# leejeongho3214/LightHand

Measured on AMD Instinct MI355X. Metric: images/sec/GPU (256×256, bs=64) train+infer; EPE/AUC parity, higher is better.
Workload: dtype bf16; 1 GPU; SimpleBaseline-ResNet50 256x256 training step (fwd + JointsMSELoss + argmax decode + bwd + Adam), batch 64/GPU, 21 joints, random init (seed 9001), hipGraph replay; global_batch=64, parallelism=dp1

## Files before the change

include/lighthand_hip.h:

```cpp
#ifndef LIGHTHAND_HIP_H
#define LIGHTHAND_HIP_H

#include <stddef.h>
#include <stdint.h>

#ifdef __cplusplus
extern "C" {
#endif

typedef enum { LH_F32 = 0, LH_BF16 = 1, LH_F16 = 2 } lh_dtype;

typedef enum {
    LH_OK = 0,
    LH_ERR_ARG = -1,
    LH_ERR_HIP = -2,
    LH_ERR_UNSUPPORTED = -3
} lh_status;

int lh_version(void);
const char* lh_last_error(void);
int lh_dtype_size(int dtype);

int lh_image_to_nhwc4(const float* nchw, void* out, int n, int h, int w, int pad, int wp,
                      int dtype, void* stream);
int lh_image_u8_to_nhwc4(const unsigned char* hwc, void* out, int n, int hs, int ws, int h, int w, int pad, int wp,
                         const float* mean3, const float* std3, int dtype, void* stream);
size_t lh_image_jitter_workspace_bytes(int n);
int lh_image_u8_jitter_to_nhwc4(const unsigned char* hwc, void* out, int n, int hs, int ws, int h, int w, int pad, int wp,
                                const float* mean3, const float* std3, const float* factors_dev, const int* order_dev,
                                void* workspace, int dtype, void* stream);
int lh_image_u8_warp_to_nhwc4(const unsigned char* hwc, void* out, int n, int hs, int ws, int h, int w, int pad, int wp,
                              const float* mean3, const float* std3, const float* inv_dev,
                              const float* factors_dev, const int* order_dev, void* workspace, int dtype, void* stream);
int lh_affine_points(const float* pts, int pstride, const float* fwd_dev, float* out, int ostride, int b, int j, void* stream);
int lh_nhwc4_mirror(void* img, int n, int h, int w, int pad, int wp, int dtype, void* stream);
int lh_nhwc_to_nchw_f32(const void* nhwc, float* nchw, int n, int h, int w, int c, int c_stride,
                        int dtype, void* stream);
int lh_nchw_f32_to_nhwc(const float* nchw, void* nhwc, int n, int h, int w, int c, int c_stride,
                        int dtype, void* stream);

int lh_pack_weight(const float* w, void* out, size_t* bytes, int n_out, int n_in,
                   long so, long si, long sr, long ss, int ntaps, const int* taps_rs,
                   int dtype, void* stream);

typedef struct {
    const float* w;
    void* out;
    int n_out, n_in, ntaps, pad_;
    long so, si, sr, ss;
    signed char r[64];
    signed char s[64];
} lh_pack_item;
int lh_pack_chunk_elems(void);
int lh_pack_weights_multi(const lh_pack_item* items_dev, const int* chunk_item_dev, const long* chunk_start_dev,
                          int n_chunks, int dtype, void* stream);

typedef struct {
    void* out;
    int row_is_d1, ntaps, kpad, pad_;
    int taps[16];
} lh_pack_out;
typedef struct {
    const float* w;
    int d0, d1, rs, npacks;
    lh_pack_out packs[5];
} lh_pack_conv;
int lh_pack_weights_tiled(const lh_pack_conv* convs_dev, const int* chunk_conv_dev, const int* chunk_t0_dev,
                          const int* chunk_t1_dev, int n_chunks, int max_rs, int dtype, void* stream);

typedef struct {
    int n, hi, wi;
    int in_pix_stride;
    int k_run;
    int ho, wo;
    int sh, sw;
    int cout;
    int OH, OW;
    int osh, osw, ooh, oow;
    int out_pix_stride;
    int ntaps;
    int relu;
    signed char dh[64];
    signed char dw[64];
    int cfg[8];
} lh_igemm_desc;

int lh_igemm(const lh_igemm_desc* d, const void* in, const void* wpack, void* out,
             const void* addend, const void* addend_mask, const float* bias, const float* scale, const float* shift,
             float* stats, int dtype, void* stream);
typedef struct {
    const void* x;
    const float* mean;
    const float* invstd;
    const float* scale;
    const float* shift;
    float* partial;
    const void* mask;
    const void* x2;
    const float* mean2;
    const float* invstd2;
    float* partial2;
} lh_bn_bwd_gate;
int lh_igemm_gated_rows(const lh_igemm_desc* d, int dtype, int nterms);
int lh_igemm_gated(const lh_igemm_desc* d, const void* in, const void* wpack, void* out, const void* addend, const void* addend_mask,
                   const lh_bn_bwd_gate* gate, int dtype, void* stream);
int lh_igemm_phases_rows(const lh_igemm_desc* const* descs, int nphase, int dtype);
int lh_igemm_phases(const lh_igemm_desc* const* descs, int nphase, const void* in, const void* const* wpacks,
                    void* out, const void* addend, const void* addend_mask, const float* bias, const float* scale,
                    const float* shift, float* stats, int dtype, void* stream);
typedef struct {
    const void* w;
    size_t w_row_bytes;
    const float* bias;
    float* out;
    int n_out;
} lh_head;
int lh_igemm_phases_head(const lh_igemm_desc* const* descs, int nphase, const void* in, const void* const* wpacks,
                         const float* scale, const float* shift, const lh_head* head, int dtype, void* stream);
int lh_igemm_tile(const lh_igemm_desc* d, int dtype, int* bm, int* bp, int* ring);
int lh_igemm_config(const lh_igemm_desc* d, int dtype, int* cfg5);
int lh_igemm_candidates(const lh_igemm_desc* d, int dtype, int* cfgs, int max);
int lh_wgrad_rowfold(const lh_igemm_desc* d, int rows, const void* x, const void* dy, int dy_pix_stride,
                     int n_out, float* slab, int dtype, void* stream);
int lh_wgrad_tile(const lh_igemm_desc* d, int n_out, int n_in, int dtype, int* bo, int* bi, int* nsplit, int* ring);
int lh_wgrad_candidates(const lh_igemm_desc* d, int n_out, int n_in, int dtype, int* out, int max);
typedef struct {
    const lh_igemm_desc* d; const void* in; const void* wpack; void* out; const void* addend; const void* addend_mask;
    const float* bias; const float* scale; const float* shift; float* stats;
} lh_igemm_call;
int lh_igemm_multi(const lh_igemm_call* calls, int n, int dtype, void* stream);
int lh_igemm_stats_rows(const lh_igemm_desc* d, int dtype);

size_t lh_wgrad_slab_bytes(const lh_igemm_desc* d, int n_out, int n_in, int dtype);
int lh_wgrad(const lh_igemm_desc* d, const void* x, const void* dy, int dy_pix_stride,
             int n_out, int n_in, float* slab, int dtype, void* stream);
int lh_wgrad_reduce(const lh_igemm_desc* d, const float* slab, float* grad, int n_out, int n_in,
                    long so, long si, long sr, long ss, const int* taps_rs, int accumulate,
                    int dtype, void* stream);
size_t lh_wgrad_workspace_bytes(const lh_igemm_desc* d, int n_out, int n_in, int dtype);
typedef struct {
    const lh_igemm_desc* d; int rows; const void* x; const void* dy; int dy_pix_stride, n_out, n_in; void* workspace; float* grad;
    long so, si, sr, ss; const int* taps_rs; int accumulate;
} lh_wgrad_call;
int lh_wgrad_fused_multi(const lh_wgrad_call* calls, int n, int dtype, void* stream);
int lh_wgrad_fused(const lh_igemm_desc* d, int rows, const void* x, const void* dy, int dy_pix_stride, int n_out, int n_in,
                   void* workspace, float* grad, long so, long si, long sr, long ss, const int* taps_rs, int accumulate,
                   int dtype, void* stream);
typedef struct {
    int bo, bi, kps, depth;
    int n_problems, n_fold;
    int n_items, n_fold_items;
    int fold_lds, target_stages, nsplit_max;
    int run_parts;
    size_t off_items, off_fold_args, off_fold_items, table_bytes, workspace_bytes;
} lh_wgrad_table_info;
int lh_wgrad_table_build(const lh_wgrad_call* calls, int n, int dtype, const int* cfg4, int target_stages, void* workspace,
                         void* host_blob, size_t host_bytes, lh_wgrad_table_info* info);
int lh_wgrad_table_run(const void* table, const lh_wgrad_table_info* info, int dtype, void* stream);


int lh_bn_stats(const void* y, int m, int c, float* stats, int* rows_out, int dtype, void* stream);
int lh_bn_stats_rows(int m, int c);
size_t lh_bn_stats_slab_bytes(int rows, int c);
int lh_bn_finalize(const float* stats, int rows, int count, int c, const float* gamma,
                   const float* beta, float* running_mean, float* running_var,
                   long long* num_batches_tracked, float momentum, float eps, float* scale,
                   float* shift, float* save_mean, float* save_invstd, void* stream);
typedef struct {
    const float* stats; int rows, count, c; const float* gamma; const float* beta; float* running_mean; float* running_var;
    long long* num_batches_tracked; float momentum, eps; float* scale; float* shift; float* save_mean; float* save_invstd;
} lh_bn_finalize_call;
int lh_bn_finalize_multi(const lh_bn_finalize_call* calls, int n, void* stream);
int lh_bn_eval_affine(const float* gamma, const float* beta, const float* running_mean,
                      const float* running_var, float eps, int c, float* scale, float* shift,
                      void* stream);

typedef struct {
    const void* x[4];
    const float* scale[4];
    const float* shift[4];
    int log2up[4];
    int nterms;
    int relu;
    void* relu_mask;
    const lh_bn_finalize_call* fin[4];
    const void* l2_touch;
    size_t l2_touch_bytes;
} lh_fuse_desc;
int lh_fuse_fwd(const lh_fuse_desc* d, void* out, int n, int h, int w, int c, int dtype, void* stream);
typedef struct { const lh_fuse_desc* d; void* out; int n, h, w, c; } lh_fuse_fwd_call;
int lh_fuse_fwd_multi(const lh_fuse_fwd_call* calls, int n, int dtype, void* stream);

typedef struct {
    const void* dout;
    const void* out;
    const void* x[4];
    const float* scale[4];
    const float* shift[4];
    const float* save_mean[4];
    const float* save_invstd[4];
    void* dx[4];
    float* dgamma[4];
    float* dbeta[4];
    int log2up[4];
    int accumulate[4];
    int nterms;
    int relu;
    const void* relu_mask;
    int strips_cap;
    const float* pre_partial;
    int pre_rows;
    const void* l2_touch;
    size_t l2_touch_bytes;
    const float* pre_partial2;
} lh_fuse_bwd_desc;
size_t lh_fuse_bwd_workspace_bytes(int n, int h, int w, int c);
int lh_fuse_bwd(const lh_fuse_bwd_desc* d, int n, int h, int w, int c, void* workspace,
                int dtype, void* stream);
typedef struct { const lh_fuse_bwd_desc* d; int n, h, w, c; void* workspace; } lh_fuse_bwd_call;
int lh_fuse_bwd_multi(const lh_fuse_bwd_call* calls, int n, int dtype, void* stream);

int lh_stem_pool(const void* img, int n, int hp, int wp, const void* wpack, const float* bias, const float* scale,
                 const float* shift, void* out, int conv_h, int conv_w, int relu, int dtype, void* stream);

typedef struct { int n, h, w, cin, mid, cout; } lh_bottleneck_desc;
int lh_bottleneck_infer(const lh_bottleneck_desc* d, const void* x, const void* w1, const void* w2, const void* w3,
                        const float* s1, const float* b1, const float* s2, const float* b2, const float* s3, const float* b3,
                        const void* residual, void* out, int dtype, void* stream);

int lh_stem_conv_rows(int n, int conv_h, int conv_w);
int lh_stem_conv(const void* img, int n, int hp, int wp, const void* wpack, void* out, float* stats, int conv_h, int conv_w,
                 int dtype, void* stream);

int lh_maxpool3x3s2_fwd(const void* x, void* out, unsigned char* idx, int n, int h, int w, int c,
                        int dtype, void* stream);
int lh_maxpool3x3s2_bwd(const void* dout, const unsigned char* idx, void* dx, int n, int h, int w,
                        int c, int dtype, void* stream);
int lh_maxpool3x3s2_bwd_gated_rows(int n, int h, int w, int c, int dtype);
int lh_maxpool3x3s2_bwd_gated(const void* dout, const unsigned char* idx, void* dx, const lh_bn_bwd_gate* gate, int n, int h, int w,
                              int c, int dtype, void* stream);
int lh_bn_relu_maxpool3x3s2_fwd(const void* x, const float* scale, const float* shift, void* out, unsigned char* idx, int n,
                                int h, int w, int c, int dtype, void* stream);

int lh_gaussian_target(const float* joints, int jstride, const float* patch, int radius,
                       float* target, int b, int j, int size, void* stream);
int lh_gaussian_target_alt(const float* points, int pstride, const float* patch, int sigma,
                           float* target, int b, int j, int res, void* stream);
size_t lh_mse_workspace_bytes(long numel);
int lh_mse_heatmap(const float* pred, const float* target, long numel, float* loss, float* grad,
                   const float* grad_scale, void* workspace, void* stream);
int lh_gaussian_target_w(const float* joints, int jstride, const float* vis, int vstride, const float* patch, int radius,
                         float* target, float* weight, int b, int j, int size, void* stream);
int lh_gaussian_target_sub(const float* joints, int jstride, const float* vis, int vstride, int radius, float sigma,
                           float* target, float* weight, int b, int j, int size, void* stream);
size_t lh_joints_mse_workspace_bytes(int b, int j);
int lh_joints_mse(const float* pred, const float* target, const float* weight, int b, int j, int hw, int topk, float* loss,
                  float* joint_loss, float* grad, const float* grad_scale, void* workspace, void* stream);
int lh_heatmap_argmax(const float* heatmaps, int bj, int h, int w, float scale, float* preds,
                      float* maxvals, int* idx, void* stream);
int lh_heatmap_soft_argmax(const float* heatmaps, int bj, int h, int w, float beta, float scale, float* preds,
                           void* stream);
int lh_heatmap_refine(const float* heatmaps, const int* idx, const float* maxvals, int bj, int h, int w,
                      float scale, float* preds, void* stream);
size_t lh_integral_l1_workspace_bytes(int b, int j);
int lh_integral_l1(const float* heatmaps, const float* joints, int jstride, const float* weight, int b, int j, int h, int w,
                   float beta, float scale, float lambda, float* preds, float* joint_loss, float* loss, int add_to_loss,
                   float* grad, int add_to_grad, const float* grad_scale, void* workspace, void* stream);
int lh_heatmap_dark(const float* heatmaps, const int* idx, const float* maxvals, int bj, int h, int w, int blur_kernel,
                    float scale, float* preds, void* stream);
int lh_heatmap_flip_merge(const float* a, const float* m, int bj, int h, int w, int shift, float scale, float* merged,
                          float* preds, float* maxvals, int* idx, void* stream);

int lh_keypoint_metrics(const float* pred, const float* gt, int gt_stride, int b, int j, float T, int* wrong,
                        float* epe, void* stream);

int lh_adam_step(float* param, const float* grad, float* exp_avg, float* exp_avg_sq, long numel,
                 const double* hyper, int* step, float* derived, float grad_scale, void* stream);
int lh_adam_tick(const double* hyper, int* step, float* derived, void* stream);
int lh_adam_apply(float* param, const float* grad, float* exp_avg, float* exp_avg_sq, long numel, const float* derived,
                  float grad_scale, void* stream);

int lh_amp_check_blocks(void);
int lh_amp_check(const float* grad, long numel, int* partial, void* stream);
int lh_amp_update(const int* partial, const double* amp_hyper, float* scale, int* growth_tracker, int* found_inf, int* skipped,
                  float* inv, double extra, const double* hyper, int* step, float* derived, void* stream);
int lh_adam_apply_guarded(float* param, const float* grad, float* exp_avg, float* exp_avg_sq, long numel, const float* derived,
                          const int* found_inf, const float* inv, void* stream);

size_t lh_channel_sum_workspace_bytes(int c);
int lh_channel_sum_nchw(const float* x, int n, int c, int hw, float* out, void* workspace, void* stream);

int lh_channel_sum_nhwc(const void* x, long pixels, int c, int pix_stride, float* out, void* workspace, int dtype, void* stream);

int lh_pck_curve(const float* pred, const float* gt, int gt_stride, const float* bb, int n, int j, const double* thr,
                 int nthr, unsigned long long* counts, unsigned long long* nvis, double* diff_row, void* stream);

typedef struct lh_comm lh_comm;
int lh_comm_unique_id(void* id128);
int lh_comm_init(lh_comm** comm, int rank, int nranks, const void* id128);
int lh_comm_allreduce_sum(lh_comm* comm, void* buf, size_t count, int dtype, void* stream);
int lh_comm_reduce_scatter_sum(lh_comm* comm, const void* send, void* recv, size_t count, int dtype, void* stream);
int lh_comm_allgather(lh_comm* comm, const void* send, void* recv, size_t count, int dtype, void* stream);
int lh_comm_alltoall(lh_comm* comm, const void* send, void* recv, size_t count, int dtype, void* stream);
int lh_comm_size(const lh_comm* comm, int* rank, int* nranks);
int lh_comm_destroy(lh_comm* comm);

int lh_copy_strided_f32(float* dst, const float* src, const int* shape4, const long* dst_strides4, const long* src_strides4,
                        void* stream);


int lh_cast_f32_bf16(float* f32, void* b16, long n, int to_f32, void* stream);

int lh_sum_chunks(const void* in, void* out, int rows, long len, int dtype, void* stream);

#ifdef __cplusplus
}
#endif
#endif
```

lighthand_amd/_lib.py:

```python
import ctypes as C
import os

_HERE = os.path.dirname(os.path.abspath(__file__))
LIB_PATH = os.environ.get("LH_LIB_PATH") or os.path.join(_HERE, "liblighthand_hip.so")

LH_F32, LH_BF16, LH_F16 = 0, 1, 2


class LightHandError(RuntimeError):
    pass


class IgemmDesc(C.Structure):
    _fields_ = [("n", C.c_int), ("hi", C.c_int), ("wi", C.c_int), ("in_pix_stride", C.c_int),
                ("k_run", C.c_int), ("ho", C.c_int), ("wo", C.c_int), ("sh", C.c_int), ("sw", C.c_int),
                ("cout", C.c_int), ("OH", C.c_int), ("OW", C.c_int), ("osh", C.c_int), ("osw", C.c_int),
                ("ooh", C.c_int), ("oow", C.c_int), ("out_pix_stride", C.c_int), ("ntaps", C.c_int),
                ("relu", C.c_int), ("dh", C.c_byte * 64), ("dw", C.c_byte * 64), ("cfg", C.c_int * 8)]


class BnFinalizeCall(C.Structure):
    _fields_ = [("stats", C.c_void_p), ("rows", C.c_int), ("count", C.c_int), ("c", C.c_int), ("gamma", C.c_void_p), ("beta", C.c_void_p),
                ("running_mean", C.c_void_p), ("running_var", C.c_void_p), ("num_batches_tracked", C.c_void_p), ("momentum", C.c_float),
                ("eps", C.c_float), ("scale", C.c_void_p), ("shift", C.c_void_p), ("save_mean", C.c_void_p), ("save_invstd", C.c_void_p)]


class FuseDesc(C.Structure):
    _fields_ = [("x", C.c_void_p * 4), ("scale", C.c_void_p * 4), ("shift", C.c_void_p * 4),
                ("log2up", C.c_int * 4), ("nterms", C.c_int), ("relu", C.c_int), ("relu_mask", C.c_void_p),
                ("fin", C.POINTER(BnFinalizeCall) * 4), ("l2_touch", C.c_void_p), ("l2_touch_bytes", C.c_size_t)]


class FuseBwdDesc(C.Structure):
    _fields_ = [("dout", C.c_void_p), ("out", C.c_void_p), ("x", C.c_void_p * 4), ("scale", C.c_void_p * 4),
                ("shift", C.c_void_p * 4), ("save_mean", C.c_void_p * 4), ("save_invstd", C.c_void_p * 4), ("dx", C.c_void_p * 4),
                ("dgamma", C.c_void_p * 4), ("dbeta", C.c_void_p * 4), ("log2up", C.c_int * 4),
                ("accumulate", C.c_int * 4), ("nterms", C.c_int), ("relu", C.c_int),
                ("relu_mask", C.c_void_p), ("strips_cap", C.c_int), ("pre_partial", C.c_void_p), ("pre_rows", C.c_int),
                ("l2_touch", C.c_void_p), ("l2_touch_bytes", C.c_size_t), ("pre_partial2", C.c_void_p)]


class BnBwdGate(C.Structure):
    _fields_ = [("x", C.c_void_p), ("mean", C.c_void_p), ("invstd", C.c_void_p), ("scale", C.c_void_p), ("shift", C.c_void_p),
                ("partial", C.c_void_p), ("mask", C.c_void_p), ("x2", C.c_void_p), ("mean2", C.c_void_p), ("invstd2", C.c_void_p), ("partial2", C.c_void_p)]


class IgemmCall(C.Structure):
    _fields_ = [("d", C.POINTER(IgemmDesc)), ("in_", C.c_void_p), ("wpack", C.c_void_p), ("out", C.c_void_p), ("addend", C.c_void_p),
                ("addend_mask", C.c_void_p), ("bias", C.c_void_p), ("scale", C.c_void_p), ("shift", C.c_void_p), ("stats", C.c_void_p)]


class WgradCall(C.Structure):
    _fields_ = [("d", C.POINTER(IgemmDesc)), ("rows", C.c_int), ("x", C.c_void_p), ("dy", C.c_void_p), ("dy_pix_stride", C.c_int),
                ("n_out", C.c_int), ("n_in", C.c_int), ("workspace", C.c_void_p), ("grad", C.c_void_p), ("so", C.c_long), ("si", C.c_long),
                ("sr", C.c_long), ("ss", C.c_long), ("taps_rs", C.POINTER(C.c_int)), ("accumulate", C.c_int)]


class WgradTableInfo(C.Structure):
    _fields_ = [("bo", C.c_int), ("bi", C.c_int), ("kps", C.c_int), ("depth", C.c_int), ("n_problems", C.c_int), ("n_fold", C.c_int),
                ("n_items", C.c_int), ("n_fold_items", C.c_int), ("fold_lds", C.c_int), ("target_stages", C.c_int), ("nsplit_max", C.c_int),
                ("run_parts", C.c_int), ("off_items", C.c_size_t), ("off_fold_args", C.c_size_t), ("off_fold_items", C.c_size_t),
                ("table_bytes", C.c_size_t), ("workspace_bytes", C.c_size_t)]


class FuseFwdCall(C.Structure):
    _fields_ = [("d", C.POINTER(FuseDesc)), ("out", C.c_void_p), ("n", C.c_int), ("h", C.c_int), ("w", C.c_int), ("c", C.c_int)]


class FuseBwdCall(C.Structure):
    _fields_ = [("d", C.POINTER(FuseBwdDesc)), ("n", C.c_int), ("h", C.c_int), ("w", C.c_int), ("c", C.c_int), ("workspace", C.c_void_p)]


class BottleneckDesc(C.Structure):
    _fields_ = [("n", C.c_int), ("h", C.c_int), ("w", C.c_int), ("cin", C.c_int), ("mid", C.c_int), ("cout", C.c_int)]


class Head(C.Structure):
    _fields_ = [("w", C.c_void_p), ("w_row_bytes", C.c_size_t), ("bias", C.c_void_p), ("out", C.c_void_p), ("n_out", C.c_int)]


class PackItem(C.Structure):
    _fields_ = [("w", C.c_void_p), ("out", C.c_void_p), ("n_out", C.c_int), ("n_in", C.c_int), ("ntaps", C.c_int),
                ("pad_", C.c_int), ("so", C.c_long), ("si", C.c_long), ("sr", C.c_long), ("ss", C.c_long),
                ("r", C.c_byte * 64), ("s", C.c_byte * 64)]


class PackOut(C.Structure):
    _fields_ = [("out", C.c_void_p), ("row_is_d1", C.c_int), ("ntaps", C.c_int), ("kpad", C.c_int), ("pad_", C.c_int),
                ("taps", C.c_int * 16)]


class PackConv(C.Structure):
    _fields_ = [("w", C.c_void_p), ("d0", C.c_int), ("d1", C.c_int), ("rs", C.c_int), ("npacks", C.c_int),
                ("packs", PackOut * 5)]


_P, _I, _L, _F, _SZ = C.c_void_p, C.c_int, C.c_long, C.c_float, C.c_size_t

SIGNATURES = {
    "lh_version": (_I, []),
    "lh_last_error": (C.c_char_p, []),
    "lh_dtype_size": (_I, [_I]),
    "lh_image_to_nhwc4": (_I, [_P, _P, _I, _I, _I, _I, _I, _I, _P]),
    "lh_image_u8_to_nhwc4": (_I, [_P, _P, _I, _I, _I, _I, _I, _I, _I, C.POINTER(C.c_float), C.POINTER(C.c_float), _I, _P]),
    "lh_image_jitter_workspace_bytes": (_SZ, [_I]),
    "lh_image_u8_jitter_to_nhwc4": (_I, [_P, _P, _I, _I, _I, _I, _I, _I, _I, C.POINTER(C.c_float), C.POINTER(C.c_float), _P, _P, _P, _I, _P]),
    "lh_image_u8_warp_to_nhwc4": (_I, [_P, _P, _I, _I, _I, _I, _I, _I, _I, C.POINTER(C.c_float), C.POINTER(C.c_float), _P, _P, _P, _P, _I, _P]),
    "lh_affine_points": (_I, [_P, _I, _P, _P, _I, _I, _I, _P]),
    "lh_nhwc4_mirror": (_I, [_P, _I, _I, _I, _I, _I, _I, _P]),
    "lh_nhwc_to_nchw_f32": (_I, [_P, _P, _I, _I, _I, _I, _I, _I, _P]),
    "lh_nchw_f32_to_nhwc": (_I, [_P, _P, _I, _I, _I, _I, _I, _I, _P]),
    "lh_pack_weight": (_I, [_P, _P, C.POINTER(_SZ), _I, _I, _L, _L, _L, _L, _I, C.POINTER(_I), _I, _P]),
    "lh_pack_chunk_elems": (_I, []),
    "lh_pack_weights_multi": (_I, [_P, _P, _P, _I, _I, _P]),
    "lh_pack_weights_tiled": (_I, [_P, _P, _P, _P, _I, _I, _I, _P]),
    "lh_igemm": (_I, [C.POINTER(IgemmDesc), _P, _P, _P, _P, _P, _P, _P, _P, _P, _I, _P]),
    "lh_igemm_multi": (_I, [C.POINTER(IgemmCall), _I, _I, _P]),
    "lh_igemm_phases_rows": (_I, [C.POINTER(C.POINTER(IgemmDesc)), _I, _I]),
    "lh_igemm_phases": (_I, [C.POINTER(C.POINTER(IgemmDesc)), _I, _P, C.POINTER(C.c_void_p), _P, _P, _P, _P, _P, _P, _P, _I, _P]),
    "lh_igemm_phases_head": (_I, [C.POINTER(C.POINTER(IgemmDesc)), _I, _P, C.POINTER(C.c_void_p), _P, _P, C.POINTER(Head), _I, _P]),
    "lh_igemm_tile": (_I, [C.POINTER(IgemmDesc), _I, C.POINTER(_I), C.POINTER(_I), C.POINTER(_I)]),
    "lh_igemm_config": (_I, [C.POINTER(IgemmDesc), _I, C.POINTER(_I)]),
    "lh_igemm_candidates": (_I, [C.POINTER(IgemmDesc), _I, C.POINTER(_I), _I]),
    "lh_wgrad_tile": (_I, [C.POINTER(IgemmDesc), _I, _I, _I, C.POINTER(_I), C.POINTER(_I), C.POINTER(_I), C.POINTER(_I)]),
    "lh_wgrad_candidates": (_I, [C.POINTER(IgemmDesc), _I, _I, _I, C.POINTER(_I), _I]),
    "lh_igemm_stats_rows": (_I, [C.POINTER(IgemmDesc), _I]),
    "lh_igemm_gated_rows": (_I, [C.POINTER(IgemmDesc), _I, _I]),
    "lh_igemm_gated": (_I, [C.POINTER(IgemmDesc), _P, _P, _P, _P, _P, C.POINTER(BnBwdGate), _I, _P]),
    "lh_wgrad_slab_bytes": (_SZ, [C.POINTER(IgemmDesc), _I, _I, _I]),
    "lh_wgrad": (_I, [C.POINTER(IgemmDesc), _P, _P, _I, _I, _I, _P, _I, _P]),
    "lh_wgrad_rowfold": (_I, [C.POINTER(IgemmDesc), _I, _P, _P, _I, _I, _P, _I, _P]),
    "lh_wgrad_workspace_bytes": (_SZ, [C.POINTER(IgemmDesc), _I, _I, _I]),
    "lh_wgrad_fused": (_I, [C.POINTER(IgemmDesc), _I, _P, _P, _I, _I, _I, _P, _P, _L, _L, _L, _L, C.POINTER(_I), _I, _I, _P]),
    "lh_wgrad_fused_multi": (_I, [C.POINTER(WgradCall), _I, _I, _P]),
    "lh_wgrad_table_build": (_I, [C.POINTER(WgradCall), _I, _I, C.POINTER(_I), _I, _P, _P, _SZ, C.POINTER(WgradTableInfo)]),
    "lh_wgrad_table_run": (_I, [_P, C.POINTER(WgradTableInfo), _I, _P]),
    "lh_wgrad_reduce": (_I, [C.POINTER(IgemmDesc), _P, _P, _I, _I, _L, _L, _L, _L, C.POINTER(_I), _I, _I, _P]),
    "lh_bn_stats": (_I, [_P, _I, _I, _P, C.POINTER(_I), _I, _P]),
    "lh_bn_stats_rows": (_I, [_I, _I]),
    "lh_bn_stats_slab_bytes": (_SZ, [_I, _I]),
    "lh_bn_finalize": (_I, [_P, _I, _I, _I, _P, _P, _P, _P, _P, _F, _F, _P, _P, _P, _P, _P]),
    "lh_bn_finalize_multi": (_I, [C.POINTER(BnFinalizeCall), _I, _P]),
    "lh_bn_eval_affine": (_I, [_P, _P, _P, _P, _F, _I, _P, _P, _P]),
    "lh_fuse_fwd": (_I, [C.POINTER(FuseDesc), _P, _I, _I, _I, _I, _I, _P]),
    "lh_fuse_fwd_multi": (_I, [C.POINTER(FuseFwdCall), _I, _I, _P]),
    "lh_fuse_bwd_multi": (_I, [C.POINTER(FuseBwdCall), _I, _I, _P]),
    "lh_fuse_bwd_workspace_bytes": (_SZ, [_I, _I, _I, _I]),
    "lh_fuse_bwd": (_I, [C.POINTER(FuseBwdDesc), _I, _I, _I, _I, _P, _I, _P]),
    "lh_stem_pool": (_I, [_P, _I, _I, _I, _P, _P, _P, _P, _P, _I, _I, _I, _I, _P]),
    "lh_bottleneck_infer": (_I, [C.POINTER(BottleneckDesc), _P, _P, _P, _P, _P, _P, _P, _P, _P, _P, _P, _P, _I, _P]),
    "lh_stem_conv_rows": (_I, [_I, _I, _I]),
    "lh_stem_conv": (_I, [_P, _I, _I, _I, _P, _P, _P, _I, _I, _I, _P]),
    "lh_maxpool3x3s2_fwd": (_I, [_P, _P, _P, _I, _I, _I, _I, _I, _P]),
    "lh_maxpool3x3s2_bwd": (_I, [_P, _P, _P, _I, _I, _I, _I, _I, _P]),
    "lh_bn_relu_maxpool3x3s2_fwd": (_I, [_P, _P, _P, _P, _P, _I, _I, _I, _I, _I, _P]),
    "lh_maxpool3x3s2_bwd_gated_rows": (_I, [_I, _I, _I, _I, _I]),
    "lh_maxpool3x3s2_bwd_gated": (_I, [_P, _P, _P, C.POINTER(BnBwdGate), _I, _I, _I, _I, _I, _P]),
    "lh_gaussian_target": (_I, [_P, _I, _P, _I, _P, _I, _I, _I, _P]),
    "lh_gaussian_target_alt": (_I, [_P, _I, _P, _I, _P, _I, _I, _I, _P]),
    "lh_mse_workspace_bytes": (_SZ, [_L]),
    "lh_mse_heatmap": (_I, [_P, _P, _L, _P, _P, _P, _P, _P]),
    "lh_gaussian_target_w": (_I, [_P, _I, _P, _I, _P, _I, _P, _P, _I, _I, _I, _P]),
    "lh_gaussian_target_sub": (_I, [_P, _I, _P, _I, _I, _F, _P, _P, _I, _I, _I, _P]),
    "lh_joints_mse_workspace_bytes": (_SZ, [_I, _I]),
    "lh_joints_mse": (_I, [_P, _P, _P, _I, _I, _I, _I, _P, _P, _P, _P, _P, _P]),
    "lh_heatmap_argmax": (_I, [_P, _I, _I, _I, _F, _P, _P, _P, _P]),
    "lh_channel_sum_workspace_bytes": (C.c_size_t, [_I]),
    "lh_channel_sum_nchw": (_I, [_P, _I, _I, _I, _P, _P, _P]),
    "lh_channel_sum_nhwc": (_I, [_P, C.c_long, _I, _I, _P, _P, _I, _P]),
    "lh_copy_strided_f32": (_I, [_P, _P, _P, _P, _P, _P]),
    "lh_pck_curve": (_I, [_P, _P, _I, _P, _I, _I, _P, _I, _P, _P, _P, _P]),
    "lh_heatmap_soft_argmax": (_I, [_P, _I, _I, _I, _F, _F, _P, _P]),
    "lh_heatmap_refine": (_I, [_P, _P, _P, _I, _I, _I, _F, _P, _P]),
    "lh_heatmap_dark": (_I, [_P, _P, _P, _I, _I, _I, _I, _F, _P, _P]),
    "lh_integral_l1_workspace_bytes": (_SZ, [_I, _I]),
    "lh_integral_l1": (_I, [_P, _P, _I, _P, _I, _I, _I, _I, _F, _F, _F, _P, _P, _P, _I, _P, _I, _P, _P, _P]),
    "lh_heatmap_flip_merge": (_I, [_P, _P, _I, _I, _I, _I, _F, _P, _P, _P, _P, _P]),
    "lh_keypoint_metrics": (_I, [_P, _P, _I, _I, _I, _F, _P, _P, _P]),
    "lh_comm_unique_id": (_I, [_P]),
    "lh_comm_init": (_I, [C.POINTER(_P), _I, _I, _P]),
    "lh_comm_allreduce_sum": (_I, [_P, _P, _SZ, _I, _P]),
    "lh_comm_reduce_scatter_sum": (_I, [_P, _P, _P, _SZ, _I, _P]),
    "lh_comm_allgather": (_I, [_P, _P, _P, _SZ, _I, _P]),
    "lh_comm_alltoall": (_I, [_P, _P, _P, _SZ, _I, _P]),
    "lh_comm_size": (_I, [_P, C.POINTER(_I), C.POINTER(_I)]),
    "lh_comm_destroy": (_I, [_P]),
    "lh_cast_f32_bf16": (_I, [_P, _P, _L, _I, _P]),
    "lh_sum_chunks": (_I, [_P, _P, _I, _L, _I, _P]),
    "lh_adam_step": (_I, [_P, _P, _P, _P, _L, _P, _P, _P, _F, _P]),
    "lh_adam_tick": (_I, [_P, _P, _P, _P]),
    "lh_adam_apply": (_I, [_P, _P, _P, _P, _L, _P, _F, _P]),
    "lh_amp_check_blocks": (_I, []),
    "lh_amp_check": (_I, [_P, _L, _P, _P]),
    "lh_amp_update": (_I, [_P, _P, _P, _P, _P, _P, _P, C.c_double, _P, _P, _P, _P]),
    "lh_adam_apply_guarded": (_I, [_P, _P, _P, _P, _L, _P, _P, _P, _P]),
}

_lib = None


def load():
    global _lib
    if _lib is not None:
        return _lib
    import torch
    if not os.path.exists(LIB_PATH):
        raise LightHandError(
            f"{LIB_PATH} not found: the HIP extension is the only backend of lighthand_amd "
            "(no CPU fallback). Build it with `make -C lighthand_amd/csrc`.")
    lib = C.CDLL(LIB_PATH)
    for name, (res, args) in SIGNATURES.items():
        fn = getattr(lib, name)
        fn.restype = res
        fn.argtypes = args
    _lib = lib
    return lib


def check(rc, what=""):
    if rc != 0:
        msg = load().lh_last_error().decode("utf-8", "replace")
        raise LightHandError(f"{what or 'liblighthand_hip'} failed (status {rc}): {msg}")


def dtype_code(torch_dtype):
    import torch
    return {torch.float32: LH_F32, torch.bfloat16: LH_BF16, torch.float16: LH_F16}[torch_dtype]
```

lighthand_amd/csrc/pack.hip:

```cpp
#include "common.h"

struct PackArgs {
    const float* w;
    void* out;
    int n_out, n_in, ntaps, kpad, rows;
    long so, si, sr, ss;
    signed char r[64];
    signed char s[64];
};

template <typename T>
__global__ void pack_weight_kernel(const PackArgs p) {
    const long total = (long)p.rows * p.ntaps * p.kpad;
    T* out = (T*)p.out;
    for (long i = (long)blockIdx.x * blockDim.x + threadIdx.x; i < total; i += (long)gridDim.x * blockDim.x) {
        const int k = (int)(i % p.kpad);
        const long t2 = i / p.kpad;
        const int t = (int)(t2 % p.ntaps), o = (int)(t2 / p.ntaps);
        float v = 0.f;
        if (o < p.n_out && k < p.n_in) v = p.w[o * p.so + k * p.si + p.r[t] * p.sr + p.s[t] * p.ss];
        out[i] = from_f<T>(v);
    }
}

extern "C" int lh_pack_weight(const float* w, void* out, size_t* bytes, int n_out, int n_in, long so, long si,
                              long sr, long ss, int ntaps, const int* taps_rs, int dtype, void* stream) {
    const int es = lh_dtype_size(dtype);
    LH_REQUIRE(es > 0, "lh_pack_weight: bad dtype %d", dtype);
    LH_REQUIRE(n_out > 0 && n_in > 0 && ntaps >= 0 && ntaps <= 64, "lh_pack_weight: bad sizes");
    const int kstep = 128 / es;
    const int kpad = (n_in + kstep - 1) / kstep * kstep;
    const int rows = (n_out + 127) / 128 * 128;
    const size_t need = (size_t)rows * (ntaps > 0 ? ntaps : 1) * kpad * es;
    if (bytes) *bytes = need;
    if (!out) return LH_OK;
    if (ntaps == 0) return LH_OK;
    LH_REQUIRE(w && taps_rs, "lh_pack_weight: null pointer");
    PackArgs a;
    a.w = w; a.out = out; a.n_out = n_out; a.n_in = n_in; a.ntaps = ntaps; a.kpad = kpad; a.rows = rows;
    a.so = so; a.si = si; a.sr = sr; a.ss = ss;
    for (int t = 0; t < 64; ++t) {
        a.r[t] = t < ntaps ? (signed char)taps_rs[2 * t] : 0;
        a.s[t] = t < ntaps ? (signed char)taps_rs[2 * t + 1] : 0;
    }
    const long total = (long)rows * ntaps * kpad;
    const int grid = lh_grid(total, 4096);
    LH_DISPATCH_DTYPE(dtype, T, hipLaunchKernelGGL((pack_weight_kernel<T>), dim3(grid), dim3(256), 0, (hipStream_t)stream, a));
    LH_LAUNCH_CHECK("pack_weight launch");
    return LH_OK;
}

constexpr int PACK_CHUNK = 2048;

template <typename T>
__global__ __launch_bounds__(256) void pack_weight_multi_kernel(const lh_pack_item* items, const int* chunk_item,
                                                                const long* chunk_start) {
    const lh_pack_item& p = items[chunk_item[blockIdx.x]];
    const int es = sizeof(T);
    const int kstep = 128 / es;
    const int kpad = (p.n_in + kstep - 1) / kstep * kstep;
    const int rows = (p.n_out + 127) / 128 * 128;
    const long total = (long)rows * p.ntaps * kpad;
    const long begin = chunk_start[blockIdx.x];
    long end = begin + PACK_CHUNK;
    if (end > total) end = total;
    T* out = (T*)p.out;
    for (long i = begin + threadIdx.x; i < end; i += 256) {
        const int k = (int)(i % kpad);
        const long t2 = i / kpad;
        const int t = (int)(t2 % p.ntaps), o = (int)(t2 / p.ntaps);
        float v = 0.f;
        if (o < p.n_out && k < p.n_in) v = p.w[o * p.so + k * p.si + p.r[t] * p.sr + p.s[t] * p.ss];
        out[i] = from_f<T>(v);
    }
}

extern "C" int lh_pack_chunk_elems(void) { return PACK_CHUNK; }

extern "C" int lh_pack_weights_multi(const lh_pack_item* items_dev, const int* chunk_item_dev, const long* chunk_start_dev,
                                     int n_chunks, int dtype, void* stream) {
    LH_REQUIRE(items_dev && chunk_item_dev && chunk_start_dev && n_chunks > 0, "lh_pack_weights_multi: bad arguments");
    LH_DISPATCH_DTYPE(dtype, T, hipLaunchKernelGGL((pack_weight_multi_kernel<T>), dim3(n_chunks), dim3(256), 0, (hipStream_t)stream,
                                                   items_dev, chunk_item_dev, chunk_start_dev));
    LH_LAUNCH_CHECK("pack_weights_multi launch");
    return LH_OK;
}

template <typename T>
__global__ __launch_bounds__(256) void pack_tiled_kernel(const lh_pack_conv* convs, const int* chunk_conv, const int* chunk_t0,
                                                         const int* chunk_t1) {
    extern __shared__ __attribute__((aligned(16))) unsigned char psm[];
    T* tile = reinterpret_cast<T*>(psm);
    const lh_pack_conv& c = convs[chunk_conv[blockIdx.x]];
    const int t0 = chunk_t0[blockIdx.x] * 32, t1 = chunk_t1[blockIdx.x] * 32;
    const int rs = c.rs;
    const int rowlen = 32 * rs;
    const int ld = rowlen + 4;
    const bool full = t0 + 32 <= c.d0 && t1 + 32 <= c.d1 && ((long)c.d1 * rs) % 4 == 0 && sizeof(T) == 2;
    if (full) {
        const int vpr = rowlen / 4;
        for (int i = threadIdx.x; i < 32 * vpr; i += 256) {
            const int a = i / vpr, v4 = i - a * vpr;
            const float4 v = *reinterpret_cast<const float4*>(c.w + ((long)(t0 + a) * c.d1 + t1) * rs + v4 * 4);
            union { uint2 u; T e[4]; } pk;
            pk.e[0] = from_f<T>(v.x); pk.e[1] = from_f<T>(v.y); pk.e[2] = from_f<T>(v.z); pk.e[3] = from_f<T>(v.w);
            *reinterpret_cast<uint2*>(tile + a * ld + v4 * 4) = pk.u;
        }
    } else {
        for (int i = threadIdx.x; i < 32 * rowlen; i += 256) {
            const int a = i / rowlen, rem = i - a * rowlen;
            const int d0 = t0 + a, d1 = t1 + rem / rs;
            float v = 0.f;
            if (d0 < c.d0 && d1 < c.d1) v = c.w[((long)d0 * c.d1 + t1) * rs + rem];
            tile[a * ld + rem] = from_f<T>(v);
        }
    }
    __syncthreads();
    for (int p = 0; p < c.npacks; ++p) {
        const lh_pack_out& o = c.packs[p];
        T* out = reinterpret_cast<T*>(o.out);
        const int nrow = o.row_is_d1 ? c.d1 : c.d0, nk = o.row_is_d1 ? c.d0 : c.d1;
        const int r0 = o.row_is_d1 ? t1 : t0, k0 = o.row_is_d1 ? t0 : t1;
        if (full && (o.kpad & 3) == 0) {
            const int total = o.ntaps * 32 * 8;
            for (int i = threadIdx.x; i < total; i += 256) {
                const int k = (i & 7) * 4, rest = i >> 3;
                const int t = rest % o.ntaps, row = rest / o.ntaps;
                const int tap = o.taps[t];
                union { uint2 u; T e[4]; } pk;
#pragma unroll
                for (int e = 0; e < 4; ++e)
                    pk.e[e] = o.row_is_d1 ? tile[(k + e) * ld + row * rs + tap] : tile[row * ld + (k + e) * rs + tap];
                *reinterpret_cast<uint2*>(out + ((long)(r0 + row) * o.ntaps + t) * o.kpad + k0 + k) = pk.u;
            }
            continue;
        }
        const int total = o.ntaps * 32 * 32;
        for (int i = threadIdx.x; i < total; i += 256) {
            const int k = i & 31, rest = i >> 5;
            const int t = rest % o.ntaps, row = rest / o.ntaps;
            const int tap = o.taps[t];
            int a, b;
            if (o.row_is_d1) { b = row; a = k; } else { a = row; b = k; }
            const int grow = r0 + row, gk = k0 + k;
            if (grow < nrow && gk < nk) out[((long)grow * o.ntaps + t) * o.kpad + gk] = tile[a * ld + b * rs + tap];
        }
    }
}

extern "C" int lh_pack_weights_tiled(const lh_pack_conv* convs_dev, const int* chunk_conv_dev, const int* chunk_t0_dev,
                                     const int* chunk_t1_dev, int n_chunks, int max_rs, int dtype, void* stream) {
    LH_REQUIRE(convs_dev && chunk_conv_dev && chunk_t0_dev && chunk_t1_dev && n_chunks > 0 && max_rs > 0 && max_rs <= 49,
               "lh_pack_weights_tiled: bad arguments");
    const int es = lh_dtype_size(dtype);
    const size_t lds = (size_t)32 * (32 * max_rs + 4) * es;
    LH_REQUIRE(lds <= 64 * 1024, "lh_pack_weights_tiled: tile of %d taps does not fit LDS for this dtype", max_rs);
    LH_DISPATCH_DTYPE(dtype, T, hipLaunchKernelGGL((pack_tiled_kernel<T>), dim3(n_chunks), dim3(256), lds, (hipStream_t)stream,
                                                   convs_dev, chunk_conv_dev, chunk_t0_dev, chunk_t1_dev));
    LH_LAUNCH_CHECK("pack_weights_tiled launch");
    return LH_OK;
}
```

Baseline: 7476 images/s.

## Batch tiled weight packing into runs with prefetched float4 loads and wide stores

Reworks the tiled weight-pack kernel so each block handles a run of up to four chunks. Adjacent chunks of the same conv are merged into wider tiles, and the next tile's float4 global loads are issued while the current tile is being written out. Fast-path stores now use 16-byte uint4 writes, and the conv descriptor is staged in LDS. The generic gather pack kernels gain an LDS-staged path that keeps reads coalesced when the input stride is the larger one. The cost is more register pressure (18 float4 per thread), more LDS, and a second launch for the leftover chunks. Weight packing is a small part of the training step, so the overall effect is probably small.

Result: no change. 7479 images/s (median of 5 runs) (+0.0%).

```diff
diff --git a/include/lighthand_hip.h b/include/lighthand_hip.h
--- a/include/lighthand_hip.h
+++ b/include/lighthand_hip.h
@@ -67,6 +67,7 @@
 } lh_pack_conv;
 int lh_pack_weights_tiled(const lh_pack_conv* convs_dev, const int* chunk_conv_dev, const int* chunk_t0_dev,
                           const int* chunk_t1_dev, int n_chunks, int max_rs, int dtype, void* stream);
+int lh_pack_tile_run(void);
 
 typedef struct {
     int n, hi, wi;
diff --git a/lighthand_amd/_lib.py b/lighthand_amd/_lib.py
--- a/lighthand_amd/_lib.py
+++ b/lighthand_amd/_lib.py
@@ -114,6 +114,7 @@
     "lh_pack_chunk_elems": (_I, []),
     "lh_pack_weights_multi": (_I, [_P, _P, _P, _I, _I, _P]),
     "lh_pack_weights_tiled": (_I, [_P, _P, _P, _P, _I, _I, _I, _P]),
+    "lh_pack_tile_run": (_I, []),
     "lh_igemm": (_I, [C.POINTER(IgemmDesc), _P, _P, _P, _P, _P, _P, _P, _P, _P, _I, _P]),
     "lh_igemm_multi": (_I, [C.POINTER(IgemmCall), _I, _I, _P]),
     "lh_igemm_phases_rows": (_I, [C.POINTER(C.POINTER(IgemmDesc)), _I, _I]),
diff --git a/lighthand_amd/csrc/pack.hip b/lighthand_amd/csrc/pack.hip
--- a/lighthand_amd/csrc/pack.hip
+++ b/lighthand_amd/csrc/pack.hip
@@ -9,17 +9,72 @@
     signed char s[64];
 };
 
+constexpr int PACK_CHUNK = 2048;
+constexpr int PACK_PER_THREAD = PACK_CHUNK / 256;
+static_assert(PACK_PER_THREAD * 256 == PACK_CHUNK, "a chunk is a whole number of elements per thread");
+
+template <typename T, typename G>
+__device__ __forceinline__ void pack_gather_chunk(const G& g, int kpad, long begin, long end, T* stage) {
+    const float* __restrict__ w = g.w;
+    T* __restrict__ out = (T*)g.out;
+    const int ntaps = g.ntaps, n_out = g.n_out, n_in = g.n_in;
+    const long so = g.so, si = g.si, sr = g.sr, ss = g.ss;
+    const int tid = threadIdx.x;
+    if (si <= so) {
+        float v[PACK_PER_THREAD];
+#pragma unroll
+        for (int u = 0; u < PACK_PER_THREAD; ++u) {
+            const long i = begin + tid + 256 * u;
+            const int k = (int)(i % kpad);
+            const long t2 = i / kpad;
+            const int t = (int)(t2 % ntaps), o = (int)(t2 / ntaps);
+            v[u] = 0.f;
+            if (i < end && o < n_out && k < n_in) v[u] = w[o * so + k * si + g.r[t] * sr + g.s[t] * ss];
+        }
+#pragma unroll
+        for (int u = 0; u < PACK_PER_THREAD; ++u) {
+            const long i = begin + tid + 256 * u;
+            if (i < end) out[i] = from_f<T>(v[u]);
+        }
+        return;
+    }
+    const long r0 = begin / kpad;
+    const int nr = (int)((end - 1) / kpad - r0) + 1;
+    const int box = nr * kpad;
+    for (int j0 = 0; j0 < box; j0 += PACK_CHUNK) {
+        float v[PACK_PER_THREAD];
+        int dst[PACK_PER_THREAD];
+#pragma unroll
+        for (int u = 0; u < PACK_PER_THREAD; ++u) {
+            const int j = j0 + tid + 256 * u;
+            const int k = j / nr;
+            const long line = r0 + (j - k * nr);
+            const long i = line * kpad + k;
+            const int t = (int)(line % ntaps), o = (int)(line / ntaps);
+            v[u] = 0.f;
+            dst[u] = j < box && i >= begin && i < end ? (int)(i - begin) : -1;
+            if (dst[u] >= 0 && o < n_out && k < n_in) v[u] = w[o * so + k * si + g.r[t] * sr + g.s[t] * ss];
+        }
+#pragma unroll
+        for (int u = 0; u < PACK_PER_THREAD; ++u)
+            if (dst[u] >= 0) stage[dst[u]] = from_f<T>(v[u]);
+    }
+    __syncthreads();
+#pragma unroll
+    for (int u = 0; u < PACK_PER_THREAD; ++u) {
+        const long i = begin + tid + 256 * u;
+        if (i < end) out[i] = stage[i - begin];
+    }
+}
+
 template <typename T>
-__global__ void pack_weight_kernel(const PackArgs p) {
+__global__ __launch_bounds__(256) void pack_weight_kernel(const PackArgs p) {
+    __shared__ T stage[PACK_CHUNK];
     const long total = (long)p.rows * p.ntaps * p.kpad;
-    T* out = (T*)p.out;
-    for (long i = (long)blockIdx.x * blockDim.x + threadIdx.x; i < total; i += (long)gridDim.x * blockDim.x) {
-        const int k = (int)(i % p.kpad);
-        const long t2 = i / p.kpad;
-        const int t = (int)(t2 % p.ntaps), o = (int)(t2 / p.ntaps);
-        float v = 0.f;
-        if (o < p.n_out && k < p.n_in) v = p.w[o * p.so + k * p.si + p.r[t] * p.sr + p.s[t] * p.ss];
-        out[i] = from_f<T>(v);
+    for (long begin = (long)blockIdx.x * PACK_CHUNK; begin < total; begin += (long)gridDim.x * PACK_CHUNK) {
+        const long end = begin + PACK_CHUNK < total ? begin + PACK_CHUNK : total;
+        pack_gather_chunk<T>(p, p.kpad, begin, end, stage);
+        __syncthreads();
     }
 }
 
@@ -44,17 +99,17 @@
         a.s[t] = t < ntaps ? (signed char)taps_rs[2 * t + 1] : 0;
     }
     const long total = (long)rows * ntaps * kpad;
-    const int grid = lh_grid(total, 4096);
+    const long chunks = (total + PACK_CHUNK - 1) / PACK_CHUNK;
+    const int grid = (int)(chunks > 1024 ? 1024 : chunks);
     LH_DISPATCH_DTYPE(dtype, T, hipLaunchKernelGGL((pack_weight_kernel<T>), dim3(grid), dim3(256), 0, (hipStream_t)stream, a));
     LH_LAUNCH_CHECK("pack_weight launch");
     return LH_OK;
 }
 
-constexpr int PACK_CHUNK = 2048;
-
 template <typename T>
-__global__ __launch_bounds__(256) void pack_weight_multi_kernel(const lh_pack_item* items, const int* chunk_item,
-                                                                const long* chunk_start) {
+__global__ __launch_bounds__(256) void pack_weight_multi_kernel(const lh_pack_item* __restrict__ items, const int* __restrict__ chunk_item,
+                                                                const long* __restrict__ chunk_start) {
+    __shared__ T stage[PACK_CHUNK];
     const lh_pack_item& p = items[chunk_item[blockIdx.x]];
     const int es = sizeof(T);
     const int kstep = 128 / es;
@@ -64,15 +119,7 @@
     const long begin = chunk_start[blockIdx.x];
     long end = begin + PACK_CHUNK;
     if (end > total) end = total;
-    T* out = (T*)p.out;
-    for (long i = begin + threadIdx.x; i < end; i += 256) {
-        const int k = (int)(i % kpad);
-        const long t2 = i / kpad;
-        const int t = (int)(t2 % p.ntaps), o = (int)(t2 / p.ntaps);
-        float v = 0.f;
-        if (o < p.n_out && k < p.n_in) v = p.w[o * p.so + k * p.si + p.r[t] * p.sr + p.s[t] * p.ss];
-        out[i] = from_f<T>(v);
-    }
+    pack_gather_chunk<T>(p, kpad, begin, end, stage);
 }
 
 extern "C" int lh_pack_chunk_elems(void) { return PACK_CHUNK; }
@@ -86,77 +133,190 @@
     return LH_OK;
 }
 
+constexpr int PACK_RUN = 4;
+constexpr int PACK_FUSE_K = 18;
+constexpr int PACK_LD_PAD = 8;
+
+struct PackEntry {
+    const float* w;
+    int ci, t0, t1, d0, d1, rs;
+    int ok, pad_;
+};
+
+struct PackFill {
+    const float* w;
+    int ci, d0, d1, rs, t0, t1;
+    int nt, lg;
+    int next;
+    int fast;
+};
+
 template <typename T>
-__global__ __launch_bounds__(256) void pack_tiled_kernel(const lh_pack_conv* convs, const int* chunk_conv, const int* chunk_t0,
-                                                         const int* chunk_t1) {
+__device__ __forceinline__ PackEntry pack_entry(const lh_pack_conv* __restrict__ convs, const int* __restrict__ chunk_conv,
+                                                const int* __restrict__ chunk_t0, const int* __restrict__ chunk_t1, int i) {
+    PackEntry e;
+    e.ci = chunk_conv[i]; e.t0 = chunk_t0[i]; e.t1 = chunk_t1[i];
+    const lh_pack_conv& c = convs[e.ci];
+    e.w = c.w; e.d0 = c.d0; e.d1 = c.d1; e.rs = c.rs; e.pad_ = 0;
+    bool ok = sizeof(T) == 2 && c.rs <= PACK_FUSE_K && ((long)c.d1 * c.rs) % 4 == 0 && ((size_t)c.w & 15) == 0 &&
+              e.t0 * 32 + 32 <= c.d0 && e.t1 * 32 + 32 <= c.d1;
+#pragma unroll
+    for (int p = 0; p < 5; ++p)
+        if (p < c.npacks) ok = ok && (c.packs[p].kpad & 7) == 0 && ((size_t)c.packs[p].out & 15) == 0;
+    e.ok = ok;
+    return e;
+}
+
+__device__ __forceinline__ PackFill pack_scan(const PackEntry* srun, int i, int cnt) {
+    const PackEntry h = srun[i];
+    PackFill f;
+    f.w = h.w; f.ci = h.ci; f.d0 = h.d0; f.d1 = h.d1; f.rs = h.rs; f.t0 = h.t0 * 32; f.t1 = h.t1 * 32;
+    f.nt = 1; f.lg = 2; f.fast = h.ok;
+    if (h.ok) {
+        const int want = h.rs <= 2 ? 8 : h.rs <= 4 ? 4 : h.rs <= 9 ? 2 : 1;
+        int n = 1;
+        while (n < want && i + n < cnt && srun[i + n].ok && srun[i + n].ci == h.ci && srun[i + n].t0 == h.t0 && srun[i + n].t1 == h.t1 + n)
+            ++n;
+        while (f.nt * 2 <= n) { f.nt *= 2; ++f.lg; }
+    }
+    f.next = i + f.nt;
+    return f;
+}
+
+__device__ __forceinline__ void pack_issue(const PackFill& f, float4 (&v)[PACK_FUSE_K]) {
+    const int a = threadIdx.x >> 3, l = threadIdx.x & 7, nv = f.nt * f.rs;
+    const float* src = f.w + ((long)(f.t0 + a) * f.d1 + f.t1) * f.rs + l * 4;
+#pragma unroll
+    for (int j = 0; j < PACK_FUSE_K; ++j)
+        if (j < nv) v[j] = *reinterpret_cast<const float4*>(src + 32 * j);
+}
+
+template <typename T>
+__global__ __launch_bounds__(256) void pack_tiled_kernel(const lh_pack_conv* __restrict__ convs, const int* __restrict__ chunk_conv,
+                                                         const int* __restrict__ chunk_t0, const int* __restrict__ chunk_t1) {
     extern __shared__ __attribute__((aligned(16))) unsigned char psm[];
+    __shared__ __attribute__((aligned(16))) int sdesc[sizeof(lh_pack_conv) / sizeof(int)];
     T* tile = reinterpret_cast<T*>(psm);
-    const lh_pack_conv& c = convs[chunk_conv[blockIdx.x]];
-    const int t0 = chunk_t0[blockIdx.x] * 32, t1 = chunk_t1[blockIdx.x] * 32;
-    const int rs = c.rs;
-    const int rowlen = 32 * rs;
-    const int ld = rowlen + 4;
-    const bool full = t0 + 32 <= c.d0 && t1 + 32 <= c.d1 && ((long)c.d1 * rs) % 4 == 0 && sizeof(T) == 2;
-    if (full) {
-        const int vpr = rowlen / 4;
-        for (int i = threadIdx.x; i < 32 * vpr; i += 256) {
-            const int a = i / vpr, v4 = i - a * vpr;
-            const float4 v = *reinterpret_cast<const float4*>(c.w + ((long)(t0 + a) * c.d1 + t1) * rs + v4 * 4);
-            union { uint2 u; T e[4]; } pk;
-            pk.e[0] = from_f<T>(v.x); pk.e[1] = from_f<T>(v.y); pk.e[2] = from_f<T>(v.z); pk.e[3] = from_f<T>(v.w);
-            *reinterpret_cast<uint2*>(tile + a * ld + v4 * 4) = pk.u;
-        }
-    } else {
-        for (int i = threadIdx.x; i < 32 * rowlen; i += 256) {
-            const int a = i / rowlen, rem = i - a * rowlen;
-            const int d0 = t0 + a, d1 = t1 + rem / rs;
-            float v = 0.f;
-            if (d0 < c.d0 && d1 < c.d1) v = c.w[((long)d0 * c.d1 + t1) * rs + rem];
-            tile[a * ld + rem] = from_f<T>(v);
-        }
-    }
+    const lh_pack_conv& c = *reinterpret_cast<const lh_pack_conv*>(sdesc);
+    const int tid = threadIdx.x;
+    __shared__ __attribute__((aligned(16))) PackEntry srun[PACK_RUN];
+    const bool whole = gridDim.y == 1;
+    if (!whole && blockIdx.y + 1 == gridDim.y) return;
+    const int first = whole ? ((int)gridDim.x - 1 - (int)blockIdx.x) * PACK_RUN : (int)blockIdx.y;
+    const int end = whole ? PACK_RUN : 1;
+    if (tid < end) srun[tid] = pack_entry<T>(convs, chunk_conv, chunk_t0, chunk_t1, first + tid);
     __syncthreads();
-    for (int p = 0; p < c.npacks; ++p) {
-        const lh_pack_out& o = c.packs[p];
-        T* out = reinterpret_cast<T*>(o.out);
-        const int nrow = o.row_is_d1 ? c.d1 : c.d0, nk = o.row_is_d1 ? c.d0 : c.d1;
-        const int r0 = o.row_is_d1 ? t1 : t0, k0 = o.row_is_d1 ? t0 : t1;
-        if (full && (o.kpad & 3) == 0) {
-            const int total = o.ntaps * 32 * 8;
-            for (int i = threadIdx.x; i < total; i += 256) {
-                const int k = (i & 7) * 4, rest = i >> 3;
+    float4 v[PACK_FUSE_K];
+    PackFill cur = pack_scan(srun, 0, end);
+    if (cur.fast) pack_issue(cur, v);
+    int staged = -1;
+    for (;;) {
+        const int rs = cur.rs, t0 = cur.t0, t1 = cur.t1;
+        const int rowlen = 32 * cur.nt * rs;
+        const int ld = rowlen + PACK_LD_PAD;
+        if (cur.ci != staged) {
+            const int* g = reinterpret_cast<const int*>(convs + cur.ci);
+            if (tid < (int)(sizeof(lh_pack_conv) / sizeof(int))) sdesc[tid] = g[tid];
+            staged = cur.ci;
+        }
+        if (cur.fast) {
+            const int a = tid >> 3, l = tid & 7, nv = cur.nt * rs;
+#pragma unroll
+            for (int j = 0; j < PACK_FUSE_K; ++j)
+                if (j < nv) {
+                    union { uint2 u; T e[4]; } pk;
+                    pk.e[0] = from_f<T>(v[j].x); pk.e[1] = from_f<T>(v[j].y); pk.e[2] = from_f<T>(v[j].z); pk.e[3] = from_f<T>(v[j].w);
+                    *reinterpret_cast<uint2*>(tile + a * ld + (l + 8 * j) * 4) = pk.u;
+                }
+        } else {
+            const int d0n = cur.d0;
+            for (int i = tid; i < 32 * rowlen; i += 256) {
+                const int a = i / rowlen, rem = i - a * rowlen;
+                const int d0 = t0 + a, d1 = t1 + rem / rs;
+                float x = 0.f;
+                if (d0 < d0n && d1 < cur.d1) x = cur.w[((long)d0 * cur.d1 + t1) * rs + rem];
+                tile[a * ld + rem] = from_f<T>(x);
+            }
+        }
+        __syncthreads();
+        const bool more = cur.next < end;
+        const bool fast = cur.fast != 0;
+        const int lg = cur.lg;
+        PackFill nxt = cur;
+        if (more) {
+            nxt = pack_scan(srun, cur.next, end);
+            if (nxt.fast) pack_issue(nxt, v);
+        }
+        for (int p = 0; p < c.npacks; ++p) {
+            const lh_pack_out& o = c.packs[p];
+            T* out = reinterpret_cast<T*>(o.out);
+            if (fast) {
+                const int total = o.ntaps << (lg + 5);
+                if (!o.row_is_d1) {
+                    for (int i = tid; i < total; i += 256) {
+                        const int ch = i & ((1 << lg) - 1), row = (i >> lg) & 31, t = i >> (lg + 5);
+                        const T* s = tile + row * ld + ch * 8 * rs + o.taps[t];
+                        union { uint4 u; T e[8]; } pk;
+                        if (rs == 1) {
+                            pk.u = *reinterpret_cast<const uint4*>(s);
+                        } else {
+#pragma unroll
+                            for (int e = 0; e < 8; ++e) pk.e[e] = s[e * rs];
+                        }
+                        *reinterpret_cast<uint4*>(out + ((long)(t0 + row) * o.ntaps + t) * o.kpad + t1 + ch * 8) = pk.u;
+                    }
+                } else {
+                    for (int i = tid; i < total; i += 256) {
+                        const int k8 = i & 3, b = (i >> 2) & ((8 << lg) - 1), t = i >> (lg + 5);
+                        const T* s = tile + k8 * 8 * ld + b * rs + o.taps[t];
+                        union { uint4 u; T e[8]; } pk;
+#pragma unroll
+                        for (int e = 0; e < 8; ++e) pk.e[e] = s[e * ld];
+                        *reinterpret_cast<uint4*>(out + ((long)(t1 + b) * o.ntaps + t) * o.kpad + t0 + k8 * 8) = pk.u;
+                    }
+                }
+                continue;
+            }
+            const int nrow = o.row_is_d1 ? c.d1 : c.d0, nk = o.row_is_d1 ? c.d0 : c.d1;
+            const int r0 = o.row_is_d1 ? t1 : t0, k0 = o.row_is_d1 ? t0 : t1;
+            const int total = o.ntaps * 32 * 32;
+            for (int i = tid; i < total; i += 256) {
+                const int k = i & 31, rest = i >> 5;
                 const int t = rest % o.ntaps, row = rest / o.ntaps;
                 const int tap = o.taps[t];
-                union { uint2 u; T e[4]; } pk;
-#pragma unroll
-                for (int e = 0; e < 4; ++e)
-                    pk.e[e] = o.row_is_d1 ? tile[(k + e) * ld + row * rs + tap] : tile[row * ld + (k + e) * rs + tap];
-                *reinterpret_cast<uint2*>(out + ((long)(r0 + row) * o.ntaps + t) * o.kpad + k0 + k) = pk.u;
+                int a, b;
+                if (o.row_is_d1) { b = row; a = k; } else { a = row; b = k; }
+                const int grow = r0 + row, gk = k0 + k;
+                if (grow < nrow && gk < nk) out[((long)grow * o.ntaps + t) * o.kpad + gk] = tile[a * ld + b * rs + tap];
             }
-            continue;
-        }
-        const int total = o.ntaps * 32 * 32;
-        for (int i = threadIdx.x; i < total; i += 256) {
-            const int k = i & 31, rest = i >> 5;
-            const int t = rest % o.ntaps, row = rest / o.ntaps;
-            const int tap = o.taps[t];
-            int a, b;
-            if (o.row_is_d1) { b = row; a = k; } else { a = row; b = k; }
-            const int grow = r0 + row, gk = k0 + k;
-            if (grow < nrow && gk < nk) out[((long)grow * o.ntaps + t) * o.kpad + gk] = tile[a * ld + b * rs + tap];
-        }
-    }
-}
+        }
+        if (!more) break;
+        __syncthreads();
+        cur = nxt;
+    }
+}
+
+extern "C" int lh_pack_tile_run(void) { return PACK_RUN; }
 
 extern "C" int lh_pack_weights_tiled(const lh_pack_conv* convs_dev, const int* chunk_conv_dev, const int* chunk_t0_dev,
                                      const int* chunk_t1_dev, int n_chunks, int max_rs, int dtype, void* stream) {
     LH_REQUIRE(convs_dev && chunk_conv_dev && chunk_t0_dev && chunk_t1_dev && n_chunks > 0 && max_rs > 0 && max_rs <= 49,
                "lh_pack_weights_tiled: bad arguments");
     const int es = lh_dtype_size(dtype);
-    const size_t lds = (size_t)32 * (32 * max_rs + 4) * es;
-    LH_REQUIRE(lds <= 64 * 1024, "lh_pack_weights_tiled: tile of %d taps does not fit LDS for this dtype", max_rs);
-    LH_DISPATCH_DTYPE(dtype, T, hipLaunchKernelGGL((pack_tiled_kernel<T>), dim3(n_chunks), dim3(256), lds, (hipStream_t)stream,
-                                                   convs_dev, chunk_conv_dev, chunk_t0_dev, chunk_t1_dev));
-    LH_LAUNCH_CHECK("pack_weights_tiled launch");
+    LH_REQUIRE((size_t)32 * (32 * max_rs + 4) * es <= 64 * 1024, "lh_pack_weights_tiled: tile of %d taps does not fit LDS for this dtype", max_rs);
+    const int cap = es == 2 && max_rs < PACK_FUSE_K ? PACK_FUSE_K : max_rs;
+    const size_t lds = (size_t)32 * (32 * cap + PACK_LD_PAD) * es;
+    const int runs = n_chunks / PACK_RUN, left = n_chunks - runs * PACK_RUN;
+    if (runs > 0) {
+        LH_DISPATCH_DTYPE(dtype, T, hipLaunchKernelGGL((pack_tiled_kernel<T>), dim3(runs), dim3(256), lds, (hipStream_t)stream,
+                                                       convs_dev, chunk_conv_dev, chunk_t0_dev, chunk_t1_dev));
+        LH_LAUNCH_CHECK("pack_weights_tiled launch");
+    }
+    if (left > 0) {
+        const int at = runs * PACK_RUN;
+        LH_DISPATCH_DTYPE(dtype, T, hipLaunchKernelGGL((pack_tiled_kernel<T>), dim3(1, left + 1), dim3(256), lds, (hipStream_t)stream,
+                                                       convs_dev, chunk_conv_dev + at, chunk_t0_dev + at, chunk_t1_dev + at));
+        LH_LAUNCH_CHECK("pack_weights_tiled launch (table end)");
+    }
     return LH_OK;
 }
```
